# openfheorg/openfhe-boolean-circuit-evaluator

Hardware: AMD Instinct MI355X
Metric: encrypted gate-bootstraps/sec (whole node), AES-128 Bristol ckt STD128 GINX (higher is better)
Workload: dtype u32

## Files before the change

openfhe-boolean-circuit-evaluator_amd/csrc/kernels.hip:

```cpp
#include <hip/hip_runtime.h>

#include <algorithm>
#include <iterator>
#include <utility>

#include "kernels.hpp"

namespace bce {

#include "phase_prof.hpp"
#include "gate_front.hpp"
#include "fused_tail.hpp"
#include "dag_sched.hpp"
#ifdef BCE_PHASE_PROF
__device__ unsigned long long g_phase_prof[BCE_PROF_WAVES * BCE_PROF_SLOTS];
#define BCE_PROF_ARRAY ::bce::g_phase_prof
#endif

__device__ __forceinline__ u32 csub(u32 x, u32 m) { return min(x, x - m); }

__device__ __forceinline__ u32 mul_shoup_lazy(u32 y, uint2 w, u32 Q) {
    u32 qh = __umulhi(w.y, y);
    return w.x * y - qh * Q;
}

__device__ __forceinline__ u64 mad64(u32 a, u32 b, u64 c) {
    u64 r, carry;
    asm("v_mad_u64_u32 %0, %1, %2, %3, %4" : "=v"(r), "=s"(carry) : "v"(a), "v"(b), "v"(c));
    return r;
}
__device__ __forceinline__ u64 mul64(u32 a, u32 b) {
    u64 r, carry;
    asm("v_mad_u64_u32 %0, %1, %2, %3, 0" : "=v"(r), "=s"(carry) : "v"(a), "v"(b));
    return r;
}
__device__ __forceinline__ u32 mul_shoup_lazy3(u32 y, uint2 w, u32 Q) {
    return (u32)mad64(__umulhi(w.y, y), 0u - Q, mul64(y, w.x));
}
__device__ __forceinline__ u64 pair_of(u32 lo) {
    u64 p;
    asm volatile("" : "=v"(p));
    return (p & 0xFFFFFFFF00000000ull) | lo;
}
__device__ __forceinline__ u64 with_lo(u64 pair, u32 lo) { return (pair & 0xFFFFFFFF00000000ull) | lo; }

__device__ __forceinline__ u32 barrett_lazy3(u64 x, u32 Q, u32 shift, u32 mu) {
    return (u32)mad64(__umulhi((u32)(x >> shift), mu), 0u - Q, x);
}

__device__ __forceinline__ u32 barrett_reduce(u64 x, u32 Q, u32 shift, u32 mu) {
    u32 x1 = (u32)(x >> shift);
    u32 qh = __umulhi(x1, mu);
    u32 r = (u32)x - qh * Q;
    r = csub(r, 2 * Q);
    return csub(r, Q);
}

__device__ __forceinline__ u32 barrett_fold(u64 x, u32 c32, u32 Q, u32 shift, u32 mu) {
    return barrett_reduce((u64)(u32)(x >> 32) * c32 + (u32)x, Q, shift, mu);
}


template <int LOGN>
struct Cfg {
    static constexpr int N = 1 << LOGN;
    static constexpr int LE = LOGN - 6;
    static constexpr int E = 1 << LE;
    static constexpr int NP = N + (N >> 6) * 4;
    static constexpr int F2LO = (6 > LE) ? 6 - LE : 0;
    static_assert(LOGN >= 9 && LOGN <= 11, "supported ring sizes: 512, 1024, 2048");
};

template <u32 M>
__device__ __forceinline__ u32 tw_pos(u32 i) {
    if constexpr (M < 64) {
        return M + i;
    } else {
// ... 43 lines not shown
        uint4* p = reinterpret_cast<uint4*>(poly + phys(lane * E));
#pragma unroll
        for (int k = 0; k < E / 4; ++k) p[k] = make_uint4(x[4 * k], x[4 * k + 1], x[4 * k + 2], x[4 * k + 3]);
    } else {
#pragma unroll
        for (int r = 0; r < E; ++r) poly[phys(elem_j<LOGN, LO>(lane, r))] = x[r];
    }
}

template <int LOGN, int LO, int B, bool LAZY>
__device__ __forceinline__ void fwd_stage(u32 (&x)[Cfg<LOGN>::E], u32 lane, const uint2* tw, u32 Q) {
    constexpr int LE = Cfg<LOGN>::LE, E = Cfg<LOGN>::E;
    constexpr int rb = B - LO;
    constexpr u32 m = 1u << (LOGN - 1 - B);
    const u32 hi = (lane >> LO) << (LO + LE - B - 1);
    const u32 Q2 = 2 * Q;
#pragma unroll
    for (int r = 0; r < E; ++r) {
        if (r & (1 << rb)) continue;
        uint2 w = tw[tw_pos<m>(hi | (u32)(r >> (rb + 1)))];
        u32 X = LAZY ? x[r] : csub(x[r], Q2);
        u32 T = mul_shoup_lazy(x[r | (1 << rb)], w, Q);
        x[r] = X + T;
        x[r | (1 << rb)] = X + Q2 - T;
    }
}

template <int LOGN, int LO, int B>
__device__ __forceinline__ void fwd_stage_pair(u64 (&x)[Cfg<LOGN>::E], u32 lane, const uint2* tw, u32 Q) {
    constexpr int LE = Cfg<LOGN>::LE, E = Cfg<LOGN>::E;
    constexpr int rb = B - LO;
    constexpr u32 m = 1u << (LOGN - 1 - B);
    const u32 hi = (lane >> LO) << (LO + LE - B - 1);
    const u32 Q2 = 2 * Q, negQ = 0u - Q;
#pragma unroll
    for (int r = 0; r < E; ++r) {
        if (r & (1 << rb)) continue;
        const uint2 w = tw[tw_pos<m>(hi | (u32)(r >> (rb + 1)))];
        const u32 X = (u32)x[r], Y = (u32)x[r | (1 << rb)];
        const u64 t = mad64(__umulhi(Y, w.y), negQ, mad64(Y, w.x, x[r]));
        x[r | (1 << rb)] = with_lo(x[r | (1 << rb)], (X << 1) + Q2 - (u32)t);
        x[r] = t;
    }
}
template <int LOGN>
__device__ __forceinline__ void fwd_first_stage_pair(const u32 (&x)[Cfg<LOGN>::E], u64 (&xp)[Cfg<LOGN>::E], uint2 w, u32 Q) {
    constexpr int E = Cfg<LOGN>::E, Hh = E / 2;
    const u32 Q2 = 2 * Q, negQ = 0u - Q;
#pragma unroll
    for (int r = 0; r < Hh; ++r) {
        const u32 X = x[r], Y = x[r + Hh];
        const u64 t = mad64(__umulhi(Y, w.y), negQ, mad64(Y, w.x, pair_of(X)));
        xp[r] = t;
        xp[r + Hh] = pair_of((X << 1) + Q2 - (u32)t);
    }
}
template <int LOGN, int LO, int BHI, int BLO>
__device__ __forceinline__ void fwd_stages_pair(u64 (&x)[Cfg<LOGN>::E], u32 lane, const uint2* tw, u32 Q) {
    if constexpr (BHI >= BLO) {
        fwd_stage_pair<LOGN, LO, BHI>(x, lane, tw, Q);
        fwd_stages_pair<LOGN, LO, BHI - 1, BLO>(x, lane, tw, Q);
    }
}
template <int LOGN, int LO>
__device__ __forceinline__ void load_pass_pair(const u32* poly, u32 lane, u64 (&x)[Cfg<LOGN>::E]) {
#pragma unroll
    for (int r = 0; r < Cfg<LOGN>::E; ++r) x[r] = pair_of(poly[phys(elem_j<LOGN, LO>(lane, r))]);
}
__device__ __forceinline__ u32 lm_word(u32 lane, int k) { return (u32)k * 256u + lane * 4u; }
template <int LOGN>
__device__ __forceinline__ void load_lm(const u32* poly, u32 lane, u32 (&x)[Cfg<LOGN>::E]) {
#pragma unroll
    for (int k = 0; k < Cfg<LOGN>::E / 4; ++k) {
        const uint4 v = *reinterpret_cast<const uint4*>(poly + lm_word(lane, k));
        x[4 * k] = v.x; x[4 * k + 1] = v.y; x[4 * k + 2] = v.z; x[4 * k + 3] = v.w;
    }
}
template <int LOGN, int LO>
__device__ __forceinline__ void store_pass_pair(u32* poly, u32 lane, const u64 (&x)[Cfg<LOGN>::E]) {
#pragma unroll
    for (int r = 0; r < Cfg<LOGN>::E; ++r) poly[phys(elem_j<LOGN, LO>(lane, r))] = (u32)x[r];
}

constexpr int GS_CAP = 16;
constexpr int gs_bound(int r, int rb0, int rb) {
    int b = 2;
    for (int s = rb0; s < rb; ++s) {
// ... 98 lines not shown
#pragma unroll
        for (int r = 0; r < C::E; ++r) {
            if constexpr (LAZY) {
                u32 v = x[r] - __umulhi(x[r], mu32) * Q;
                x[r] = csub(csub(v, 2 * Q), Q);
            } else {
                x[r] = csub(csub(x[r], 2 * Q), Q);
            }
        }
    }
    store_pass<LOGN, 0>(poly, lane, x);
    wave_sync();
}

__device__ __forceinline__ void ntt_forward_wave_low8(u32* poly, const uint2* twf, u32 lane, u32 Q) {
    constexpr int LOGN = 10;
    {
        u64 xp[16];
        load_pass_pair<LOGN, 4>(poly, lane, xp);
        fwd_stages_pair<LOGN, 4, 7, 4>(xp, lane, twf, Q);
        store_pass_pair<LOGN, 4>(poly, lane, xp);
    }
    wave_sync();
    u32 x[16];
    u64 xp[16];
    load_pass<LOGN, 0>(poly, lane, x);
    fwd_first_stage_pair<LOGN>(x, xp, twf[tw_pos<64>(lane)], Q);
    fwd_stages_pair<LOGN, 0, 2, 0>(xp, lane, twf, Q);
#pragma unroll
    for (int r = 0; r < 16; ++r) x[r] = (u32)xp[r];
    store_pass<LOGN, 0>(poly, lane, x);
    wave_sync();
}
__device__ __forceinline__ void fwd_bfly_pair(u64& xa, u64& xb, uint2 w, u32 Q) {
    const u32 X = (u32)xa, Y = (u32)xb;
    const u64 t = mad64(__umulhi(Y, w.y), 0u - Q, mad64(Y, w.x, xa));
    xb = with_lo(xb, (X << 1) + 2 * Q - (u32)t);
    xa = t;
}
__device__ __forceinline__ void ntt_forward_half_low8(u32* row, u32 h, const uint2* twf, u32 lane, u32 Q) {
    asm volatile("" : "+v"(lane));
    u64 xp[8];
    {
        const u32 l8 = lane >> 5, j0 = (h << 9) | (l8 << 8) | (lane & 31u);
        u32* const p = row + phys(j0);
#pragma unroll
        for (int r = 0; r < 8; ++r) xp[r] = pair_of(p[(r >> 1) * 68 + (r & 1) * 32]);
        const u32 i7 = (h << 1) | l8;
        const uint2 w7 = twf[tw_pos<4>(i7)];
#pragma unroll
        for (int r = 0; r < 4; ++r) fwd_bfly_pair(xp[r], xp[r + 4], w7, Q);
#pragma unroll
        for (int g = 0; g < 2; ++g) {
            const uint2 w6 = twf[tw_pos<8>((i7 << 1) | g)];
            fwd_bfly_pair(xp[4 * g], xp[4 * g + 2], w6, Q);
            fwd_bfly_pair(xp[4 * g + 1], xp[4 * g + 3], w6, Q);
        }
#pragma unroll
        for (int g = 0; g < 4; ++g) fwd_bfly_pair(xp[2 * g], xp[2 * g + 1], twf[tw_pos<16>((i7 << 2) | g)], Q);
#pragma unroll
        for (int r = 0; r < 8; ++r) p[(r >> 1) * 68 + (r & 1) * 32] = (u32)xp[r];
    }
    wave_sync();
    {
        const u32 lh = lane >> 2, j0 = (h << 9) | (lh << 5) | (lane & 3u);
        u32* const p = row + phys(j0);
#pragma unroll
        for (int r = 0; r < 8; ++r) xp[r] = pair_of(p[4 * r]);
        const u32 i4 = (h << 4) | lh;
        const uint2 w4 = twf[tw_pos<32>(i4)];
#pragma unroll
        for (int r = 0; r < 4; ++r) fwd_bfly_pair(xp[r], xp[r + 4], w4, Q);
#pragma unroll
        for (int g = 0; g < 2; ++g) {
            const uint2 w3 = twf[tw_pos<64>((i4 << 1) | g)];
            fwd_bfly_pair(xp[4 * g], xp[4 * g + 2], w3, Q);
            fwd_bfly_pair(xp[4 * g + 1], xp[4 * g + 3], w3, Q);
        }
#pragma unroll
        for (int g = 0; g < 4; ++g) fwd_bfly_pair(xp[2 * g], xp[2 * g + 1], twf[tw_pos<128>((i4 << 2) | g)], Q);
#pragma unroll
        for (int r = 0; r < 8; ++r) p[4 * r] = (u32)xp[r];
    }
    wave_sync();
    {
        const u32 j0 = (h << 9) | (lane << 3);
        uint4* const p = reinterpret_cast<uint4*>(row + phys(j0));
        const uint4 v0 = p[0], v1 = p[1];
        xp[0] = pair_of(v0.x); xp[1] = pair_of(v0.y); xp[2] = pair_of(v0.z); xp[3] = pair_of(v0.w);
        xp[4] = pair_of(v1.x); xp[5] = pair_of(v1.y); xp[6] = pair_of(v1.z); xp[7] = pair_of(v1.w);
        const u32 i1 = (((h << 6) | lane) << 1);
#pragma unroll
        for (int g = 0; g < 2; ++g) {
            const uint2 w1 = twf[tw_pos<256>(i1 | g)];
            fwd_bfly_pair(xp[4 * g], xp[4 * g + 2], w1, Q);
            fwd_bfly_pair(xp[4 * g + 1], xp[4 * g + 3], w1, Q);
        }
#pragma unroll
        for (int g = 0; g < 4; ++g) fwd_bfly_pair(xp[2 * g], xp[2 * g + 1], twf[tw_pos<512>((i1 << 1) | g)], Q);
        p[0] = make_uint4((u32)xp[0], (u32)xp[1], (u32)xp[2], (u32)xp[3]);
        p[1] = make_uint4((u32)xp[4], (u32)xp[5], (u32)xp[6], (u32)xp[7]);
    }
    wave_sync();
}
__device__ __forceinline__ u64 mad64_su(u32 a, u32 b_uniform, u64 c) {
    u64 r, carry;
    asm("v_mad_u64_u32 %0, %1, %2, %3, %4" : "=v"(r), "=s"(carry) : "v"(a), "s"(b_uniform), "v"(c));
    return r;
}
__device__ __forceinline__ void fwd_bfly_pair_su(u64& xa, u64& xb, uint2 w_uniform, u32 Q) {
    const u32 X = (u32)xa, Y = (u32)xb;
    const u64 t = mad64(__umulhi(Y, w_uniform.y), 0u - Q, mad64_su(Y, w_uniform.x, xa));
    xb = with_lo(xb, (X << 1) + 2 * Q - (u32)t);
    xa = t;
}
template <bool SU>
__device__ __forceinline__ void fwd_pass4_pair(u64 (&x)[4], uint2 wa, uint2 wb0, uint2 wb1, u32 Q) {
    if constexpr (SU) {
        fwd_bfly_pair_su(x[0], x[2], wa, Q); fwd_bfly_pair_su(x[1], x[3], wa, Q);
        fwd_bfly_pair_su(x[0], x[1], wb0, Q); fwd_bfly_pair_su(x[2], x[3], wb1, Q);
    } else {
        fwd_bfly_pair(x[0], x[2], wa, Q); fwd_bfly_pair(x[1], x[3], wa, Q);
        fwd_bfly_pair(x[0], x[1], wb0, Q); fwd_bfly_pair(x[2], x[3], wb1, Q);
    }
}
typedef int v4i __attribute__((ext_vector_type(4)));
__device__ __forceinline__ u32 xb_group(u32 j, u32 g) { return 64u * j + 16u * ((g ^ (0u - (j >> 2))) & 3u); }
template <bool MFMA>
__device__ __forceinline__ void ntt_forward_quarter3(u32* rows, u32 qr, uint2 w7, uint2 w6a, uint2 w6b, const u32* xb,
                                                     const v4i (&A)[4], uint2 w14, const uint2* twf, u32 lane, u32 Q) {
    constexpr int RS = 2 * Cfg<10>::NP;
    u64 xp[3][4];
    auto pass16 = [&](uint2 wa, uint2 wb0, uint2 wb1) {
        const uint4* const p = reinterpret_cast<const uint4*>(rows + 4 * lane);
        uint4 v[3];
#pragma unroll
        for (int k = 0; k < 3; ++k) v[k] = p[k * (RS / 4)];
#pragma unroll
        for (int k = 0; k < 3; ++k) {
            xp[k][0] = ((u64)v[k].y << 32) | v[k].x; xp[k][2] = pair_of(v[k].y);
            xp[k][1] = ((u64)v[k].w << 32) | v[k].z; xp[k][3] = pair_of(v[k].w);
            fwd_pass4_pair<false>(xp[k], wa, wb0, wb1, Q);
        }
    };
    auto store4 = [&](u32 off) {
        u32* const p = rows + off;
#pragma unroll
        for (int k = 0; k < 3; ++k)
#pragma unroll
            for (int r = 0; r < 4; ++r) p[k * RS + 64 * r] = (u32)xp[k][r];
    };
    if constexpr (!MFMA) {
        {
            const u32* const p = rows + lane;
#pragma unroll
            for (int k = 0; k < 3; ++k)
#pragma unroll
                for (int r = 0; r < 4; ++r) xp[k][r] = pair_of(p[k * RS + 68 * r]);
#pragma unroll
            for (int k = 0; k < 3; ++k) fwd_pass4_pair<true>(xp[k], w7, w6a, w6b, Q);
            store4(((lane & 15u) << 2) | ((lane >> 3) & 2u) | (lane >> 5));
        }
        wave_sync();
        {
            const u32 h = lane >> 4;
            const uint2 w5 = twf[tw_pos<16>(4 * qr + h)];
            const uint4 w4 = *reinterpret_cast<const uint4*>(twf + tw_pos<32>(8 * qr + 2 * h));
            pass16(w5, make_uint2(w4.x, w4.y), make_uint2(w4.z, w4.w));
            store4(((lane >> 4) << 4) | ((lane & 3u) << 2) | ((lane >> 1) & 2u) | ((lane >> 3) & 1u));
        }
        wave_sync();
        {
            const u32 h = (((lane >> 2) & 3u) << 2) | (lane >> 4);
            const uint2* const t = twf + tw_pos<64>(16 * qr + h);
            pass16(t[0], t[64], t[128]);
            store4((((lane >> 2) & 3u) << 4) | ((lane >> 4) << 2) | ((lane & 1u) << 1) | ((lane >> 1) & 1u));
        }
    } else {
        {
            const char* const pb = reinterpret_cast<const char*>(xb) + xb_group(lane & 15u, lane >> 4);
            v4i B[3];
#pragma unroll
            for (int k = 0; k < 3; ++k) B[k] = *reinterpret_cast<const v4i*>(pb + 1024 * k);
            const u32 negQ = 0u - Q;
            const v4i c0 = {(int)Q, 0, (int)Q, 0};
#pragma unroll
            for (int i = 0; i < 4; ++i) {
#pragma unroll
                for (int k = 0; k < 3; ++k) {
                    const v4i s = __builtin_amdgcn_mfma_i32_16x16x64_i8(A[i], B[k], c0, 0, 0, 0);
                    const u32 lo = ((u32)s[1] << 7) + (u32)s[0], hi = ((u32)s[3] << 7) + (u32)s[2];
                    xp[k][i] = mad64(__umulhi(hi, w14.y), negQ, mad64_su(hi, w14.x, ((u64)(u32)s[1] << 32) | lo));
                }
            }
            store4(((lane >> 4) << 4) | ((lane & 3u) << 2) | ((lane >> 1) & 2u) | ((lane >> 3) & 1u));
        }
        wave_sync();
        {
            const u32 h = lane >> 2;
            const uint2* const t = twf + tw_pos<64>(16 * qr + h);
            pass16(t[0], t[64], t[128]);
            store4((h << 2) | ((lane & 1u) << 1) | ((lane >> 1) & 1u));
        }
    }
    wave_sync();
    {
        const u32 h = lane & 15u, g = lane >> 4;
        const uint2* const t = twf + 512 + 128 * g + 16 * qr + h;
        pass16(twf[256 + 64 * g + 16 * qr + h], t[0], t[64]);
        uint4* const p = reinterpret_cast<uint4*>(rows + 16 * h + 4 * g + 4 * (h >> 2));
#pragma unroll
        for (int k = 0; k < 3; ++k) p[k * (RS / 4)] = make_uint4((u32)xp[k][0], (u32)xp[k][1], (u32)xp[k][2], (u32)xp[k][3]);
    }
    wave_sync();
}
__device__ __forceinline__ void fwd_bfly(u32& X, u32& Y, uint2 w, u32 Q) {
    const u64 t = mad64(__umulhi(Y, w.y), 0u - Q, mad64(Y, w.x, pair_of(X)));
    Y = (X << 1) + 2 * Q - (u32)t;
    X = (u32)t;
}

template <int LOGN>
__device__ __forceinline__ void ntt_inverse_wave(const u32* src, u32* tmp, const uint2* twi, u32 lane, u32 Q,
                                                 uint2 ninv, uint2 wlast, u32 mu32, u32 (&x)[Cfg<LOGN>::E]) {
    using C = Cfg<LOGN>;
    constexpr int LE = C::LE;
// ... 62 lines not shown

__device__ __forceinline__ u32 redc(u64 x, u32 Q, u32 qn) { return (u32)(mad64((u32)x * qn, Q, x) >> 32); }
template <int LOGN, bool EVENF = false, typename PT>
__device__ __forceinline__ void ginx_mac_tail_redc(const PT& P, __amdgpu_buffer_rsrc_t psi_r2_rsrc, u32 Q, u32 ap, u32 p0,
                                                   const u32* accp, u32* accw, const u64 (&sp)[4], const u64 (&sn)[4],
                                                   u32 (&a)[4]) {
    constexpr u32 N = 1u << LOGN;
    const u32 k0 = __brev(p0) >> (32 - LOGN);
    const u32 ex = ((2 * k0 + 1) * ap) & (2 * N - 1);
    const u32 off = P.r2_off, K = Q + 2 * off, qn = P.qinv_neg;
    u32 mp[4], mn[4];
    const u32 p0r = psi_pow<LOGN>(psi_r2_rsrc, ex, Q), n0r = psi_pow<LOGN>(psi_r2_rsrc, (2 * N - ex) & (2 * N - 1), Q);
    mp[0] = p0r + off;
    mn[0] = n0r + off;
    if constexpr (EVENF) {
        const bool neg = ap & 2u;
        mp[2] = neg ? K - mp[0] : mp[0];
        mn[2] = neg ? K - mn[0] : mn[0];
        mp[1] = mp[0]; mn[1] = mn[0]; mp[3] = mp[2]; mn[3] = mn[2];
    } else {
        const bool odd = ap & 1u;
        const u32 a4 = ap & 3u;
        const uint2 Ia = make_uint2(P.I4[a4], P.I4s[a4]);
        const uint2 Ina = make_uint2(P.I4[(4u - a4) & 3u], P.I4s[(4u - a4) & 3u]);
        mp[2] = csub(mul_shoup_lazy(p0r, Ia, Q), Q) + off;
        mn[2] = csub(mul_shoup_lazy(n0r, Ina, Q), Q) + off;
        mp[1] = odd ? K - mp[0] : mp[0];
        mn[1] = odd ? K - mn[0] : mn[0];
        mp[3] = odd ? K - mp[2] : mp[2];
        mn[3] = odd ? K - mn[2] : mn[2];
    }
    const uint4 a4v = *reinterpret_cast<const uint4*>(accp);
    a[0] = a4v.x; a[1] = a4v.y; a[2] = a4v.z; a[3] = a4v.w;
#pragma unroll
    for (int e = 0; e < 4; ++e) {
        const u32 rp = redc(sp[e], Q, qn), rn = redc(sn[e], Q, qn);
        a[e] = csub(redc(mad64(rn, mn[e], mul64(rp, mp[e])), Q, qn) + a[e], 2 * Q);
    }
    *reinterpret_cast<uint4*>(accw) = make_uint4(a[0], a[1], a[2], a[3]);
}

template <int LOGN, bool LAZY, u32 T, typename PT>
__device__ __forceinline__ void bootstrap_prologue(const PT& P, const bce_gate_desc& g, u32 soff, uint2* twf, u32* acc,
                                                   u32* av, u32 tid, u32 lane, u32 wave) {
    using C = Cfg<LOGN>;
    constexpr int N = C::N, NP = C::NP;
    const u32 Q = P.Q, q = P.q;
    for (u32 i = tid; i < (u32)N; i += T) twf[i] = P.tw_f[i];
    lwe_prepare<T>(P, g, soff, q, av, tid);
    __syncthreads();
    test_polynomial<T, (u32)N>(P, g.op & 0xFFu, q, av[P.n], Q, acc, acc + NP, tid);
    __syncthreads();
    if (wave == 0) ntt_forward_wave<LOGN, LAZY>(acc + NP, twf, lane, Q, P.mu32);
    __syncthreads();
}

template <int LOGN, int DG, bool LAZY, int OCC, bool AP>
__global__ __launch_bounds__(128 * DG, (OCC * 2 * DG + 3) / 4) void k_blind_rotate(
    DevParams P, const bce_gate_desc* __restrict__ descs, u32 n_desc, u32 slot_stride, u32* __restrict__ acc_out) {
    using C = Cfg<LOGN>;
    constexpr int N = C::N, NP = C::NP, E = C::E;
    constexpr u32 R = 2 * DG;
    constexpr u32 T = 64 * R;
    extern __shared__ __align__(16) u32 smem[];
    uint2* twf = reinterpret_cast<uint2*>(smem);
    u32* acc = reinterpret_cast<u32*>(twf + N);
    u32* dct = acc + 2 * NP;
    u32* av = dct + R * NP;

    const u32 tid = threadIdx.x;
    const u32 lane = tid & 63;
// ... 141 lines not shown
                const uint4 d = *reinterpret_cast<const uint4*>(dct + l * NP + pp);
                sn[0] += (u64)d.x * kB[l].x; sn[1] += (u64)d.y * kB[l].y; sn[2] += (u64)d.z * kB[l].z; sn[3] += (u64)d.w * kB[l].w;
            }
#pragma unroll
            for (u32 l = 0; l < H; ++l) {
                const uint4 d = *reinterpret_cast<const uint4*>(dct + (H + l) * NP + pp);
                sn[0] += (u64)d.x * kA[l].x; sn[1] += (u64)d.y * kA[l].y; sn[2] += (u64)d.z * kA[l].z; sn[3] += (u64)d.w * kA[l].w;
            }
            }
            u32 anew[4];
            ginx_mac_tail<LOGN, LAZY>(P, psi_rsrc, Q, ap, Ia, Ina, p0, acc + c * NP + pp, acc + c * NP + pp, sp, sn, anew);
        }
        BCE_PROF_MARK(4);
        __syncthreads();
        BCE_PROF_MARK(5);
    }
    BCE_PROF_FLUSH();

    if (wave < 2) {
        u32 x[E];
        ntt_inverse_wave<LOGN>(acc + wave * NP, dct + wave * NP, twf, lane, Q, ninv, wlast, P.mu32, x);
        u32* out = acc_out + ((size_t)blockIdx.x * 2 + wave) * N;
#pragma unroll
        for (int r = 0; r < E; ++r) out[((u32)r << 6) | lane] = x[r];
    }
}

__device__ __forceinline__ u32 xlay1(u32 p) { return (p & 15u) + 20u * ((p >> 4) & 3u) + 80u * ((p >> 6) & 3u) + 320u * (p >> 8); }
__device__ __forceinline__ u32 xlay2(u32 p) { return (p & 63u) + 80u * ((p >> 6) & 3u) + 320u * (p >> 8); }

__device__ __forceinline__ void inv_pass4(u32 (&x)[4], uint2 fa, uint2 fb, uint2 fc, u32 Q, u32 mu32) {
    const u32 Q2 = 2 * Q;
    const u32 a0 = x[0] + x[1];
    const u32 a1 = mul_shoup_lazy3(x[1] + Q2 - x[0], fa, Q);
    const u32 a2 = x[2] + x[3];
    const u32 a3 = mul_shoup_lazy3(x[3] + Q2 - x[2], fb, Q);
    const u32 b0 = a0 + a2;
    x[2] = mul_shoup_lazy3(a2 + 2 * Q2 - a0, fc, Q);
    const u32 b1 = a1 + a3;
    x[3] = mul_shoup_lazy3(a3 + Q2 - a1, fc, Q);
    x[0] = b0 - __umulhi(b0, mu32) * Q;
    x[1] = csub(b1, Q2);
}
__device__ __forceinline__ void inv_pass4_last(u32 (&x)[4], uint2 fa, uint2 fb, uint2 ninv, uint2 wlast, u32 Q) {
    const u32 Q2 = 2 * Q;
    const u32 a0 = x[0] + x[1];
    const u32 a1 = mul_shoup_lazy3(x[1] + Q2 - x[0], fa, Q);
    const u32 a2 = x[2] + x[3];
    const u32 a3 = mul_shoup_lazy3(x[3] + Q2 - x[2], fb, Q);
    x[0] = csub(mul_shoup_lazy3(a0 + a2, ninv, Q), Q);
    x[2] = csub(mul_shoup_lazy3(a0 + 2 * Q2 - a2, wlast, Q), Q);
    x[1] = csub(mul_shoup_lazy3(a1 + a3, ninv, Q), Q);
    x[3] = csub(mul_shoup_lazy3(a1 + Q2 - a3, wlast, Q), Q);
}

template <bool REGTW>
struct SplitInv {
    u32 a0, x0, l1, s1, l2, s2, l3, s3, t;
    uint2 fa[REGTW ? 5 : 1], fb[REGTW ? 5 : 1], fc[REGTW ? 4 : 1];
    u32 ia[REGTW ? 1 : 4], ic[REGTW ? 1 : 4];
};
template <bool REGTW>
__device__ __forceinline__ void split_inv_setup(SplitInv<REGTW>& S, const uint2* twf, u32 t) {
    S.t = t;
    S.a0 = phys(4 * t);
    const u32 wb = 48u * (t >> 6);
    S.x0 = S.a0 + wb;
    const u32 pb1 = ((t >> 2) << 4) | (t & 3u), pb2 = ((t >> 4) << 6) | (t & 15u), pb3 = ((t >> 6) << 8) | (t & 63u);
    S.l1 = phys(pb1) + wb; S.s1 = xlay1(pb1);
    S.l2 = xlay1(pb2); S.s2 = xlay2(pb2);
    S.l3 = xlay2(pb3); S.s3 = 320u * (t >> 6) + (t & 63u);
    const u32 u0 = t, u1 = t >> 2, u2 = t >> 4, u3 = t >> 6;
    if constexpr (REGTW) {
        S.fa[0] = twf[tw_pos<512>(511 - 2 * u0)]; S.fb[0] = twf[tw_pos<512>(510 - 2 * u0)]; S.fc[0] = twf[tw_pos<256>(255 - u0)];
        S.fa[1] = twf[tw_pos<128>(127 - 2 * u1)]; S.fb[1] = twf[tw_pos<128>(126 - 2 * u1)]; S.fc[1] = twf[tw_pos<64>(63 - u1)];
        S.fa[2] = twf[tw_pos<32>(31 - 2 * u2)];   S.fb[2] = twf[tw_pos<32>(30 - 2 * u2)];   S.fc[2] = twf[tw_pos<16>(15 - u2)];
        S.fa[3] = twf[tw_pos<8>(7 - 2 * u3)];     S.fb[3] = twf[tw_pos<8>(6 - 2 * u3)];     S.fc[3] = twf[tw_pos<4>(3 - u3)];
        S.fa[4] = twf[tw_pos<2>(1)];              S.fb[4] = twf[tw_pos<2>(0)];
    } else {
        S.ia[0] = tw_pos<512>(511 - 2 * u0); S.ic[0] = tw_pos<256>(255 - u0);
        S.ia[1] = tw_pos<128>(127 - 2 * u1); S.ic[1] = tw_pos<64>(63 - u1);
        S.ia[2] = tw_pos<32>(31 - 2 * u2);   S.ic[2] = tw_pos<16>(15 - u2);
        S.ia[3] = tw_pos<8>(7 - 2 * u3);     S.ic[3] = tw_pos<4>(3 - u3);
    }
}
template <bool REGTW, int K>
// ... 130 lines not shown
    const u32 psel0 = 0x0c0c0400u, psel1 = 0x05040100u;
    const u32 mc = tid / (N / 4), mp0 = (tid % (N / 4)) * 4, mpp = phys(mp0);
    const u32 dig0 = phys(S.t);
    const uint2 w9 = twf[1], w8a = twf[2], w8b = twf[3];
    uint2 q7 = make_uint2(0, 0), q6a = q7, q6b = q7;
    if constexpr (QUNITS && !MFMA) {
        const uint2 a = twf[tw_pos<4>(wave & 3u)], b = twf[tw_pos<8>(2 * (wave & 3u))], d = twf[tw_pos<8>(2 * (wave & 3u) + 1)];
        q7 = make_uint2(__builtin_amdgcn_readfirstlane(a.x), __builtin_amdgcn_readfirstlane(a.y));
        q6a = make_uint2(__builtin_amdgcn_readfirstlane(b.x), __builtin_amdgcn_readfirstlane(b.y));
        q6b = make_uint2(__builtin_amdgcn_readfirstlane(d.x), __builtin_amdgcn_readfirstlane(d.y));
    }
    {
        const uint4 v = *reinterpret_cast<const uint4*>(accc + S.a0);
        u32 a[4] = {v.x, v.y, v.z, v.w};
        split_pass0(S, twf, a, xa, Q, P.mu32);
    }

    BCE_PROF_INIT();
    const u32 nsteps = AP ? n * P.dR : n;
    u32 cb = 0;
    if constexpr (WPS >= 4) __builtin_amdgcn_s_setprio(2);
    for (u32 step = 0; step < nsteps; ++step) {
        u32 ap = 0, rowb;
        if constexpr (!AP) {
            ap = ginx_exponent(P, q, av[step]);
            if (ap == 0) continue;
            rowb = step * (2 * rgsw * 4);
        } else {
            const u32 i = step / P.dR, kd = step - i * P.dR;
            const u32 a0 = ap_digit(P, q, av[i], kd);
            if (a0 == 0) continue;
            rowb = (((i * P.baseR + a0) * P.dR + kd) * rgsw) * 4u;
        }
        uint4 kA[R], kB[R];
        v4i mA[4];
        auto request_rows = [&](auto kc) {
            constexpr u32 k = decltype(kc)::value - 1, G = PR / 4;
            BCE_PROF_MARK(8 + k);
#pragma unroll
            for (u32 l = k * G; l < (k + 1) * G; ++l) {
                kA[l] = bsk_row(rsrc, tid * 16u, rowb + l * (2 * N * 4));
                if constexpr (!AP) kB[l] = bsk_row(rsrc, tid * 16u, rowb + (rgsw + l * 2 * N) * 4);
            }
            if constexpr (MFMA && k == 3) {
#pragma unroll
                for (u32 v = 0; v < 4; ++v) mA[v] = __builtin_bit_cast(v4i, bsk_row(mrsrc, lane * 16u, ((wave & 3u) * 4u + v) * 1024u));
            }
        };
        {
            u32 x[4], u[4];
            split_inverse_rest(S, twf, xa, xb, Q, P.mu32, ninv, wlast, x, request_rows);
#pragma unroll
            for (int r = 0; r < 4; ++r) u[r] = x[r] + ((x[r] < Qh) ? off : offm);
            if constexpr (MFMA) {
#pragma unroll
                for (int r = 0; r < 4; ++r) u[r] ^= off;
            }
#pragma unroll
            for (u32 l = FOLD ? 1 : 0; l < (u32)DG; ++l) {
                if constexpr (MFMA) {
                    const u32 e01 = __builtin_amdgcn_perm((u32)__builtin_amdgcn_sbfe((int)u[1], l * gb, gb), (u32)__builtin_amdgcn_sbfe((int)u[0], l * gb, gb), psel0);
                    const u32 e23 = __builtin_amdgcn_perm((u32)__builtin_amdgcn_sbfe((int)u[3], l * gb, gb), (u32)__builtin_amdgcn_sbfe((int)u[2], l * gb, gb), psel0);
                    const u32 d = __builtin_amdgcn_perm(e23, e01, psel1);
                    const u32 G = S.t >> 4;
                    xbm[(3 * c + l - 1) * 256 + (xb_group(S.t & 15u, G >> 2) >> 2) + (G & 3u)] = d;
                    continue;
                }
                u32 v[4];
#pragma unroll
                for (int r = 0; r < 4; ++r) v[r] = __builtin_amdgcn_ubfe(u[r], l * gb, gb) + bias;
                fwd_bfly(v[0], v[2], w9, Q);
                fwd_bfly(v[1], v[3], w9, Q);
                fwd_bfly(v[0], v[1], w8a, Q);
                fwd_bfly(v[2], v[3], w8b, Q);
#pragma unroll
                for (int r = 0; r < 4; ++r) dct[(2 * l + c) * NP + dig0 + 272 * r] = v[r];
            }
        }
        BCE_PROF_MARK(0);
        block_sync_lds();
        BCE_PROF_MARK(1);
        if constexpr (WPS >= 4) { if (FOLD && wave >= 4) __builtin_amdgcn_s_setprio(1); else __builtin_amdgcn_s_setprio(0); }
#ifndef BCE_SKIP_FWD
        if constexpr (QUNITS) {
            ntt_forward_quarter3<MFMA>(dct + (2 + c) * NP + 272u * (wave & 3u), wave & 3u, q7, q6a, q6b, xbm + 3 * c * 256, mA,
                                       make_uint2(P.w14, P.w14s), twf, lane, Q);
        } else if constexpr (FOLD) {
            if (wave < 4) ntt_forward_wave_low8(dct + (2 + wave) * NP, twf, lane, Q);
            else ntt_forward_half_low8(dct + (6 + ((wave - 4) >> 1)) * NP, (wave - 4) & 1u, twf, lane, Q);
        } else {
            ntt_forward_wave_low8(dct + wave * NP, twf, lane, Q);
        }
#endif
        if constexpr (WPS >= 4) __builtin_amdgcn_s_setprio(2);
        BCE_PROF_MARK(2);
        if constexpr (PR < R) {
#pragma unroll
            for (u32 l = PR; l < R; ++l) kA[l] = bsk_row(rsrc, tid * 16u, rowb + l * (2 * N * 4));
#pragma unroll
            for (u32 l = PR; l < R; ++l) if constexpr (!AP) kB[l] = bsk_row(rsrc, tid * 16u, rowb + (rgsw + l * 2 * N) * 4);
        }
        block_sync_lds();
        BCE_PROF_MARK(3);
        {
            u64 sp[4] = {0, 0, 0, 0}, sn[4] = {0, 0, 0, 0};
#pragma unroll
            for (u32 l = 0; l < R; ++l) {
#ifdef BCE_SKIP_MAC
                const uint4 d = make_uint4(l + tid, l, tid, 1u);
#else
                const uint4 d = *reinterpret_cast<const uint4*>((FOLD && l < 2 ? acc + cb : dct) + l * NP + mpp);
#endif
                sp[0] += (u64)d.x * kA[l].x; sp[1] += (u64)d.y * kA[l].y; sp[2] += (u64)d.z * kA[l].z; sp[3] += (u64)d.w * kA[l].w;
                if constexpr (!AP) {
                    sn[0] += (u64)d.x * kB[l].x; sn[1] += (u64)d.y * kB[l].y; sn[2] += (u64)d.z * kB[l].z; sn[3] += (u64)d.w * kB[l].w;
                }
            }
            u32 anew[4];
            const u32* const accr = acc + cb + mc * NP + mpp;
            u32* const accw = acc + (FOLD ? 2 * NP - cb : 0) + mc * NP + mpp;
            if constexpr (AP) {
#pragma unroll
                for (int e = 0; e < 4; ++e) anew[e] = barrett_fold(sp[e], P.c32, Q, P.red_shift, P.red_mu);
                *reinterpret_cast<uint4*>(accw) = make_uint4(anew[0], anew[1], anew[2], anew[3]);
            } else {
                ginx_mac_tail_redc<LOGN, V::EVENF>(P, psi_rsrc, Q, ap, mp0, accr, accw, sp, sn, anew);
            }
            if constexpr (FOLD) cb = 2 * NP - cb;
            split_pass0(S, twf, anew, xa, Q, P.mu32);
        }
        BCE_PROF_MARK(4);
        wave_sync();
        BCE_PROF_MARK(5);
    }
    BCE_PROF_FLUSH();
    {
        u32 x[4];
        split_inverse_rest(S, twf, xa, xb, Q, P.mu32, ninv, wlast, x, [](auto) {});
        if (acc_out) {
            u32* out = acc_out + ((size_t)boot * 2 + c) * N + S.t;
#pragma unroll
            for (int r = 0; r < 4; ++r) out[256 * r] = x[r];
        }
        if constexpr (FUSE) {
#pragma unroll
            for (int r = 0; r < 4; ++r) acc[c * N + S.t + 256 * r] = x[r];
        }
    }
    if constexpr (FUSE) {
        if constexpr (WPS >= 4) __builtin_amdgcn_s_setprio(0);
        __syncthreads();
        fused_tail_outputs<T, PERSIST>(P, g, soff, acc, dct, reinterpret_cast<u64*>(dct + ((N * P.dKS + 3) & ~3u)), boot, dbg_lweN, dbg_ks);
    }
}

template <class V>
__global__ __launch_bounds__(V::T, V::WPS) void k_blind_rotate_lat(DevParams P, const bce_gate_desc* __restrict__ descs, u32 n_desc,
                                                                   u32 slot_stride, u32* __restrict__ acc_out,
                                                                   u32* __restrict__ dbg_lweN, u32* __restrict__ dbg_ks) {
    extern __shared__ __align__(16) u32 smem[];
    lat_bootstrap<V, false>(P, descs[blockIdx.x % n_desc], (blockIdx.x / n_desc) * slot_stride, blockIdx.x, smem, acc_out, dbg_lweN, dbg_ks);
}
// ... 487 lines not shown
```

Before: 193,600.

## Batch NTT butterflies into grouped multiplies for instruction-level parallelism

Replaces the inline-asm v_mad_u64_u32 helpers with plain 64-bit C multiplies, wrapped in an empty asm barrier so the 64-bit pair stays in vector registers. Forward butterflies, inverse passes and the MAC tail reduction are regrouped so that 4 or 6 independent mulhi/mad chains are issued together instead of one dependent chain at a time. The modulus is pinned to a scalar register, and a scheduling barrier is added inside the MAC loop. The aim is to hide multiply latency and let the compiler use the carry-free mad form, at the cost of higher register pressure and a possible loss of occupancy.

```diff
diff --git a/openfhe-boolean-circuit-evaluator_amd/csrc/kernels.hip b/openfhe-boolean-circuit-evaluator_amd/csrc/kernels.hip
--- a/openfhe-boolean-circuit-evaluator_amd/csrc/kernels.hip
+++ b/openfhe-boolean-circuit-evaluator_amd/csrc/kernels.hip
@@ -24,16 +24,16 @@
     return w.x * y - qh * Q;
 }
 
-__device__ __forceinline__ u64 mad64(u32 a, u32 b, u64 c) {
-    u64 r, carry;
-    asm("v_mad_u64_u32 %0, %1, %2, %3, %4" : "=v"(r), "=s"(carry) : "v"(a), "v"(b), "v"(c));
+__device__ __forceinline__ u64 keep_pair(u64 r) {
+    asm volatile("" :: "v"(r));
     return r;
 }
-__device__ __forceinline__ u64 mul64(u32 a, u32 b) {
-    u64 r, carry;
-    asm("v_mad_u64_u32 %0, %1, %2, %3, 0" : "=v"(r), "=s"(carry) : "v"(a), "v"(b));
-    return r;
-}
+__device__ __forceinline__ u64 mad64(u32 a, u32 b, u64 c) { return keep_pair((u64)a * b + c); }
+__device__ __forceinline__ u32 block_local(u32 s) {
+    asm volatile("" : "+s"(s));
+    return s;
+}
+__device__ __forceinline__ u64 mul64(u32 a, u32 b) { return (u64)a * b; }
 __device__ __forceinline__ u32 mul_shoup_lazy3(u32 y, uint2 w, u32 Q) {
     return (u32)mad64(__umulhi(w.y, y), 0u - Q, mul64(y, w.x));
 }
@@ -43,6 +43,35 @@
     return (p & 0xFFFFFFFF00000000ull) | lo;
 }
 __device__ __forceinline__ u64 with_lo(u64 pair, u32 lo) { return (pair & 0xFFFFFFFF00000000ull) | lo; }
+
+template <int K>
+__device__ __forceinline__ void mul_shoup_lazy3_group(const u32 (&y)[K], const uint2 (&w)[K], u32 Q, u32 (&r)[K]) {
+    u32 qh[K];
+    u64 t[K];
+#pragma unroll
+    for (int k = 0; k < K; ++k) qh[k] = __umulhi(w[k].y, y[k]);
+#pragma unroll
+    for (int k = 0; k < K; ++k) t[k] = mul64(y[k], w[k].x);
+#pragma unroll
+    for (int k = 0; k < K; ++k) r[k] = (u32)mad64(qh[k], 0u - Q, t[k]);
+}
+template <int K>
+__device__ __forceinline__ void fwd_bfly_group(u64* x, const int (&ia)[K], const int (&ib)[K], const uint2 (&w)[K], u32 Q) {
+    u32 qh[K];
+    u64 t[K];
+#pragma unroll
+    for (int k = 0; k < K; ++k) qh[k] = __umulhi((u32)x[ib[k]], w[k].y);
+#pragma unroll
+    for (int k = 0; k < K; ++k) t[k] = mad64((u32)x[ib[k]], w[k].x, x[ia[k]]);
+#pragma unroll
+    for (int k = 0; k < K; ++k) t[k] = mad64(qh[k], 0u - Q, t[k]);
+#pragma unroll
+    for (int k = 0; k < K; ++k) {
+        const u32 X = (u32)x[ia[k]];
+        x[ib[k]] = with_lo(x[ib[k]], (X << 1) + 2 * Q - (u32)t[k]);
+        x[ia[k]] = t[k];
+    }
+}
 
 __device__ __forceinline__ u32 barrett_lazy3(u64 x, u32 Q, u32 shift, u32 mu) {
     return (u32)mad64(__umulhi((u32)(x >> shift), mu), 0u - Q, x);
@@ -152,27 +181,42 @@
     constexpr int rb = B - LO;
     constexpr u32 m = 1u << (LOGN - 1 - B);
     const u32 hi = (lane >> LO) << (LO + LE - B - 1);
-    const u32 Q2 = 2 * Q, negQ = 0u - Q;
-#pragma unroll
-    for (int r = 0; r < E; ++r) {
-        if (r & (1 << rb)) continue;
-        const uint2 w = tw[tw_pos<m>(hi | (u32)(r >> (rb + 1)))];
-        const u32 X = (u32)x[r], Y = (u32)x[r | (1 << rb)];
-        const u64 t = mad64(__umulhi(Y, w.y), negQ, mad64(Y, w.x, x[r]));
-        x[r | (1 << rb)] = with_lo(x[r | (1 << rb)], (X << 1) + Q2 - (u32)t);
-        x[r] = t;
+    constexpr int G = E / 2 < 4 ? E / 2 : 4;
+#pragma unroll
+    for (int g = 0; g < E / 2; g += G) {
+        int ia[G], ib[G];
+        uint2 w[G];
+#pragma unroll
+        for (int k = 0; k < G; ++k) {
+            const int b = g + k;
+            const int r = ((b >> rb) << (rb + 1)) | (b & ((1 << rb) - 1));
+            ia[k] = r;
+            ib[k] = r | (1 << rb);
+            w[k] = tw[tw_pos<m>(hi | (u32)(r >> (rb + 1)))];
+        }
+        fwd_bfly_group<G>(x, ia, ib, w, Q);
     }
 }
 template <int LOGN>
 __device__ __forceinline__ void fwd_first_stage_pair(const u32 (&x)[Cfg<LOGN>::E], u64 (&xp)[Cfg<LOGN>::E], uint2 w, u32 Q) {
     constexpr int E = Cfg<LOGN>::E, Hh = E / 2;
     const u32 Q2 = 2 * Q, negQ = 0u - Q;
-#pragma unroll
-    for (int r = 0; r < Hh; ++r) {
-        const u32 X = x[r], Y = x[r + Hh];
-        const u64 t = mad64(__umulhi(Y, w.y), negQ, mad64(Y, w.x, pair_of(X)));
-        xp[r] = t;
-        xp[r + Hh] = pair_of((X << 1) + Q2 - (u32)t);
+    constexpr int G = Hh < 4 ? Hh : 4;
+#pragma unroll
+    for (int g = 0; g < Hh; g += G) {
+        u32 qh[G];
+        u64 t[G];
+#pragma unroll
+        for (int k = 0; k < G; ++k) qh[k] = __umulhi(x[g + k + Hh], w.y);
+#pragma unroll
+        for (int k = 0; k < G; ++k) t[k] = mad64(x[g + k + Hh], w.x, pair_of(x[g + k]));
+#pragma unroll
+        for (int k = 0; k < G; ++k) t[k] = mad64(qh[k], negQ, t[k]);
+#pragma unroll
+        for (int k = 0; k < G; ++k) {
+            xp[g + k] = t[k];
+            xp[g + k + Hh] = pair_of((x[g + k] << 1) + Q2 - (u32)t[k]);
+        }
     }
 }
 template <int LOGN, int LO, int BHI, int BLO>
@@ -337,12 +381,6 @@
     store_pass<LOGN, 0>(poly, lane, x);
     wave_sync();
 }
-__device__ __forceinline__ void fwd_bfly_pair(u64& xa, u64& xb, uint2 w, u32 Q) {
-    const u32 X = (u32)xa, Y = (u32)xb;
-    const u64 t = mad64(__umulhi(Y, w.y), 0u - Q, mad64(Y, w.x, xa));
-    xb = with_lo(xb, (X << 1) + 2 * Q - (u32)t);
-    xa = t;
-}
 __device__ __forceinline__ void ntt_forward_half_low8(u32* row, u32 h, const uint2* twf, u32 lane, u32 Q) {
     asm volatile("" : "+v"(lane));
     u64 xp[8];
@@ -353,16 +391,13 @@
         for (int r = 0; r < 8; ++r) xp[r] = pair_of(p[(r >> 1) * 68 + (r & 1) * 32]);
         const u32 i7 = (h << 1) | l8;
         const uint2 w7 = twf[tw_pos<4>(i7)];
-#pragma unroll
-        for (int r = 0; r < 4; ++r) fwd_bfly_pair(xp[r], xp[r + 4], w7, Q);
-#pragma unroll
-        for (int g = 0; g < 2; ++g) {
-            const uint2 w6 = twf[tw_pos<8>((i7 << 1) | g)];
-            fwd_bfly_pair(xp[4 * g], xp[4 * g + 2], w6, Q);
-            fwd_bfly_pair(xp[4 * g + 1], xp[4 * g + 3], w6, Q);
-        }
-#pragma unroll
-        for (int g = 0; g < 4; ++g) fwd_bfly_pair(xp[2 * g], xp[2 * g + 1], twf[tw_pos<16>((i7 << 2) | g)], Q);
+        fwd_bfly_group<4>(xp, {0, 1, 2, 3}, {4, 5, 6, 7}, {w7, w7, w7, w7}, Q);
+        {
+            const uint2 w6a = twf[tw_pos<8>(i7 << 1)], w6b = twf[tw_pos<8>((i7 << 1) | 1)];
+            fwd_bfly_group<4>(xp, {0, 1, 4, 5}, {2, 3, 6, 7}, {w6a, w6a, w6b, w6b}, Q);
+        }
+        fwd_bfly_group<4>(xp, {0, 2, 4, 6}, {1, 3, 5, 7}, {twf[tw_pos<16>(i7 << 2)], twf[tw_pos<16>((i7 << 2) | 1)],
+                                                           twf[tw_pos<16>((i7 << 2) | 2)], twf[tw_pos<16>((i7 << 2) | 3)]}, Q);
 #pragma unroll
         for (int r = 0; r < 8; ++r) p[(r >> 1) * 68 + (r & 1) * 32] = (u32)xp[r];
     }
@@ -374,16 +409,13 @@
         for (int r = 0; r < 8; ++r) xp[r] = pair_of(p[4 * r]);
         const u32 i4 = (h << 4) | lh;
         const uint2 w4 = twf[tw_pos<32>(i4)];
-#pragma unroll
-        for (int r = 0; r < 4; ++r) fwd_bfly_pair(xp[r], xp[r + 4], w4, Q);
-#pragma unroll
-        for (int g = 0; g < 2; ++g) {
-            const uint2 w3 = twf[tw_pos<64>((i4 << 1) | g)];
-            fwd_bfly_pair(xp[4 * g], xp[4 * g + 2], w3, Q);
-            fwd_bfly_pair(xp[4 * g + 1], xp[4 * g + 3], w3, Q);
-        }
-#pragma unroll
-        for (int g = 0; g < 4; ++g) fwd_bfly_pair(xp[2 * g], xp[2 * g + 1], twf[tw_pos<128>((i4 << 2) | g)], Q);
+        fwd_bfly_group<4>(xp, {0, 1, 2, 3}, {4, 5, 6, 7}, {w4, w4, w4, w4}, Q);
+        {
+            const uint2 w3a = twf[tw_pos<64>(i4 << 1)], w3b = twf[tw_pos<64>((i4 << 1) | 1)];
+            fwd_bfly_group<4>(xp, {0, 1, 4, 5}, {2, 3, 6, 7}, {w3a, w3a, w3b, w3b}, Q);
+        }
+        fwd_bfly_group<4>(xp, {0, 2, 4, 6}, {1, 3, 5, 7}, {twf[tw_pos<128>(i4 << 2)], twf[tw_pos<128>((i4 << 2) | 1)],
+                                                           twf[tw_pos<128>((i4 << 2) | 2)], twf[tw_pos<128>((i4 << 2) | 3)]}, Q);
 #pragma unroll
         for (int r = 0; r < 8; ++r) p[4 * r] = (u32)xp[r];
     }
@@ -395,39 +427,21 @@
         xp[0] = pair_of(v0.x); xp[1] = pair_of(v0.y); xp[2] = pair_of(v0.z); xp[3] = pair_of(v0.w);
         xp[4] = pair_of(v1.x); xp[5] = pair_of(v1.y); xp[6] = pair_of(v1.z); xp[7] = pair_of(v1.w);
         const u32 i1 = (((h << 6) | lane) << 1);
-#pragma unroll
-        for (int g = 0; g < 2; ++g) {
-            const uint2 w1 = twf[tw_pos<256>(i1 | g)];
-            fwd_bfly_pair(xp[4 * g], xp[4 * g + 2], w1, Q);
-            fwd_bfly_pair(xp[4 * g + 1], xp[4 * g + 3], w1, Q);
-        }
-#pragma unroll
-        for (int g = 0; g < 4; ++g) fwd_bfly_pair(xp[2 * g], xp[2 * g + 1], twf[tw_pos<512>((i1 << 1) | g)], Q);
+        {
+            const uint2 w1a = twf[tw_pos<256>(i1)], w1b = twf[tw_pos<256>(i1 | 1)];
+            fwd_bfly_group<4>(xp, {0, 1, 4, 5}, {2, 3, 6, 7}, {w1a, w1a, w1b, w1b}, Q);
+        }
+        fwd_bfly_group<4>(xp, {0, 2, 4, 6}, {1, 3, 5, 7}, {twf[tw_pos<512>(i1 << 1)], twf[tw_pos<512>((i1 << 1) | 1)],
+                                                           twf[tw_pos<512>((i1 << 1) | 2)], twf[tw_pos<512>((i1 << 1) | 3)]}, Q);
         p[0] = make_uint4((u32)xp[0], (u32)xp[1], (u32)xp[2], (u32)xp[3]);
         p[1] = make_uint4((u32)xp[4], (u32)xp[5], (u32)xp[6], (u32)xp[7]);
     }
     wave_sync();
 }
-__device__ __forceinline__ u64 mad64_su(u32 a, u32 b_uniform, u64 c) {
-    u64 r, carry;
-    asm("v_mad_u64_u32 %0, %1, %2, %3, %4" : "=v"(r), "=s"(carry) : "v"(a), "s"(b_uniform), "v"(c));
-    return r;
-}
-__device__ __forceinline__ void fwd_bfly_pair_su(u64& xa, u64& xb, uint2 w_uniform, u32 Q) {
-    const u32 X = (u32)xa, Y = (u32)xb;
-    const u64 t = mad64(__umulhi(Y, w_uniform.y), 0u - Q, mad64_su(Y, w_uniform.x, xa));
-    xb = with_lo(xb, (X << 1) + 2 * Q - (u32)t);
-    xa = t;
-}
-template <bool SU>
-__device__ __forceinline__ void fwd_pass4_pair(u64 (&x)[4], uint2 wa, uint2 wb0, uint2 wb1, u32 Q) {
-    if constexpr (SU) {
-        fwd_bfly_pair_su(x[0], x[2], wa, Q); fwd_bfly_pair_su(x[1], x[3], wa, Q);
-        fwd_bfly_pair_su(x[0], x[1], wb0, Q); fwd_bfly_pair_su(x[2], x[3], wb1, Q);
-    } else {
-        fwd_bfly_pair(x[0], x[2], wa, Q); fwd_bfly_pair(x[1], x[3], wa, Q);
-        fwd_bfly_pair(x[0], x[1], wb0, Q); fwd_bfly_pair(x[2], x[3], wb1, Q);
-    }
+__device__ __forceinline__ void fwd_pass4_pair3(u64 (&x)[3][4], uint2 wa, uint2 wb0, uint2 wb1, u32 Q) {
+    u64* const f = &x[0][0];
+    fwd_bfly_group<6>(f, {0, 1, 4, 5, 8, 9}, {2, 3, 6, 7, 10, 11}, {wa, wa, wa, wa, wa, wa}, Q);
+    fwd_bfly_group<6>(f, {0, 2, 4, 6, 8, 10}, {1, 3, 5, 7, 9, 11}, {wb0, wb1, wb0, wb1, wb0, wb1}, Q);
 }
 typedef int v4i __attribute__((ext_vector_type(4)));
 __device__ __forceinline__ u32 xb_group(u32 j, u32 g) { return 64u * j + 16u * ((g ^ (0u - (j >> 2))) & 3u); }
@@ -445,8 +459,8 @@
         for (int k = 0; k < 3; ++k) {
             xp[k][0] = ((u64)v[k].y << 32) | v[k].x; xp[k][2] = pair_of(v[k].y);
             xp[k][1] = ((u64)v[k].w << 32) | v[k].z; xp[k][3] = pair_of(v[k].w);
-            fwd_pass4_pair<false>(xp[k], wa, wb0, wb1, Q);
-        }
+        }
+        fwd_pass4_pair3(xp, wa, wb0, wb1, Q);
     };
     auto store4 = [&](u32 off) {
         u32* const p = rows + off;
@@ -462,8 +476,7 @@
             for (int k = 0; k < 3; ++k)
 #pragma unroll
                 for (int r = 0; r < 4; ++r) xp[k][r] = pair_of(p[k * RS + 68 * r]);
-#pragma unroll
-            for (int k = 0; k < 3; ++k) fwd_pass4_pair<true>(xp[k], w7, w6a, w6b, Q);
+            fwd_pass4_pair3(xp, w7, w6a, w6b, Q);
             store4(((lane & 15u) << 2) | ((lane >> 3) & 2u) | (lane >> 5));
         }
         wave_sync();
@@ -491,12 +504,21 @@
             const v4i c0 = {(int)Q, 0, (int)Q, 0};
 #pragma unroll
             for (int i = 0; i < 4; ++i) {
+                v4i s[3];
+                u32 hi[3], qh[3];
+                u64 t[3];
+#pragma unroll
+                for (int k = 0; k < 3; ++k) s[k] = __builtin_amdgcn_mfma_i32_16x16x64_i8(A[i], B[k], c0, 0, 0, 0);
 #pragma unroll
                 for (int k = 0; k < 3; ++k) {
-                    const v4i s = __builtin_amdgcn_mfma_i32_16x16x64_i8(A[i], B[k], c0, 0, 0, 0);
-                    const u32 lo = ((u32)s[1] << 7) + (u32)s[0], hi = ((u32)s[3] << 7) + (u32)s[2];
-                    xp[k][i] = mad64(__umulhi(hi, w14.y), negQ, mad64_su(hi, w14.x, ((u64)(u32)s[1] << 32) | lo));
+                    t[k] = ((u64)(u32)s[k][1] << 32) | (((u32)s[k][1] << 7) + (u32)s[k][0]);
+                    hi[k] = ((u32)s[k][3] << 7) + (u32)s[k][2];
+                    qh[k] = __umulhi(hi[k], w14.y);
                 }
+#pragma unroll
+                for (int k = 0; k < 3; ++k) t[k] = mad64(hi[k], w14.x, t[k]);
+#pragma unroll
+                for (int k = 0; k < 3; ++k) xp[k][i] = mad64(qh[k], negQ, t[k]);
             }
             store4(((lane >> 4) << 4) | ((lane & 3u) << 2) | ((lane >> 1) & 2u) | ((lane >> 3) & 1u));
         }
@@ -625,11 +647,16 @@
     }
     const uint4 a4v = *reinterpret_cast<const uint4*>(accp);
     a[0] = a4v.x; a[1] = a4v.y; a[2] = a4v.z; a[3] = a4v.w;
-#pragma unroll
-    for (int e = 0; e < 4; ++e) {
-        const u32 rp = redc(sp[e], Q, qn), rn = redc(sn[e], Q, qn);
-        a[e] = csub(redc(mad64(rn, mn[e], mul64(rp, mp[e])), Q, qn) + a[e], 2 * Q);
-    }
+    u32 rp[4], rn[4];
+    u64 t[4];
+#pragma unroll
+    for (int e = 0; e < 4; ++e) rp[e] = redc(sp[e], Q, qn);
+#pragma unroll
+    for (int e = 0; e < 4; ++e) rn[e] = redc(sn[e], Q, qn);
+#pragma unroll
+    for (int e = 0; e < 4; ++e) t[e] = mad64(rn[e], mn[e], mul64(rp[e], mp[e]));
+#pragma unroll
+    for (int e = 0; e < 4; ++e) a[e] = csub(redc(t[e], Q, qn) + a[e], 2 * Q);
     *reinterpret_cast<uint4*>(accw) = make_uint4(a[0], a[1], a[2], a[3]);
 }
 
@@ -837,26 +864,26 @@
 __device__ __forceinline__ void inv_pass4(u32 (&x)[4], uint2 fa, uint2 fb, uint2 fc, u32 Q, u32 mu32) {
     const u32 Q2 = 2 * Q;
     const u32 a0 = x[0] + x[1];
-    const u32 a1 = mul_shoup_lazy3(x[1] + Q2 - x[0], fa, Q);
     const u32 a2 = x[2] + x[3];
-    const u32 a3 = mul_shoup_lazy3(x[3] + Q2 - x[2], fb, Q);
+    u32 a[2], b[2];
+    mul_shoup_lazy3_group<2>({x[1] + Q2 - x[0], x[3] + Q2 - x[2]}, {fa, fb}, Q, a);
     const u32 b0 = a0 + a2;
-    x[2] = mul_shoup_lazy3(a2 + 2 * Q2 - a0, fc, Q);
-    const u32 b1 = a1 + a3;
-    x[3] = mul_shoup_lazy3(a3 + Q2 - a1, fc, Q);
+    const u32 b1 = a[0] + a[1];
+    mul_shoup_lazy3_group<2>({a2 + 2 * Q2 - a0, a[1] + Q2 - a[0]}, {fc, fc}, Q, b);
+    x[2] = b[0];
+    x[3] = b[1];
     x[0] = b0 - __umulhi(b0, mu32) * Q;
     x[1] = csub(b1, Q2);
 }
 __device__ __forceinline__ void inv_pass4_last(u32 (&x)[4], uint2 fa, uint2 fb, uint2 ninv, uint2 wlast, u32 Q) {
     const u32 Q2 = 2 * Q;
     const u32 a0 = x[0] + x[1];
-    const u32 a1 = mul_shoup_lazy3(x[1] + Q2 - x[0], fa, Q);
     const u32 a2 = x[2] + x[3];
-    const u32 a3 = mul_shoup_lazy3(x[3] + Q2 - x[2], fb, Q);
-    x[0] = csub(mul_shoup_lazy3(a0 + a2, ninv, Q), Q);
-    x[2] = csub(mul_shoup_lazy3(a0 + 2 * Q2 - a2, wlast, Q), Q);
-    x[1] = csub(mul_shoup_lazy3(a1 + a3, ninv, Q), Q);
-    x[3] = csub(mul_shoup_lazy3(a1 + Q2 - a3, wlast, Q), Q);
+    u32 a[2], r[4];
+    mul_shoup_lazy3_group<2>({x[1] + Q2 - x[0], x[3] + Q2 - x[2]}, {fa, fb}, Q, a);
+    mul_shoup_lazy3_group<4>({a0 + a2, a[0] + a[1], a0 + 2 * Q2 - a2, a[0] + Q2 - a[1]}, {ninv, ninv, wlast, wlast}, Q, r);
+#pragma unroll
+    for (int k = 0; k < 4; ++k) x[k] = csub(r[k], Q);
 }
 
 template <bool REGTW>
@@ -1053,6 +1080,7 @@
             if (a0 == 0) continue;
             rowb = (((i * P.baseR + a0) * P.dR + kd) * rgsw) * 4u;
         }
+        const u32 Qs = block_local(Q);
         uint4 kA[R], kB[R];
         v4i mA[4];
         auto request_rows = [&](auto kc) {
@@ -1070,7 +1098,7 @@
         };
         {
             u32 x[4], u[4];
-            split_inverse_rest(S, twf, xa, xb, Q, P.mu32, ninv, wlast, x, request_rows);
+            split_inverse_rest(S, twf, xa, xb, Qs, P.mu32, ninv, wlast, x, request_rows);
 #pragma unroll
             for (int r = 0; r < 4; ++r) u[r] = x[r] + ((x[r] < Qh) ? off : offm);
             if constexpr (MFMA) {
@@ -1090,10 +1118,10 @@
                 u32 v[4];
 #pragma unroll
                 for (int r = 0; r < 4; ++r) v[r] = __builtin_amdgcn_ubfe(u[r], l * gb, gb) + bias;
-                fwd_bfly(v[0], v[2], w9, Q);
-                fwd_bfly(v[1], v[3], w9, Q);
-                fwd_bfly(v[0], v[1], w8a, Q);
-                fwd_bfly(v[2], v[3], w8b, Q);
+                fwd_bfly(v[0], v[2], w9, Qs);
+                fwd_bfly(v[1], v[3], w9, Qs);
+                fwd_bfly(v[0], v[1], w8a, Qs);
+                fwd_bfly(v[2], v[3], w8b, Qs);
 #pragma unroll
                 for (int r = 0; r < 4; ++r) dct[(2 * l + c) * NP + dig0 + 272 * r] = v[r];
             }
@@ -1105,12 +1133,12 @@
 #ifndef BCE_SKIP_FWD
         if constexpr (QUNITS) {
             ntt_forward_quarter3<MFMA>(dct + (2 + c) * NP + 272u * (wave & 3u), wave & 3u, q7, q6a, q6b, xbm + 3 * c * 256, mA,
-                                       make_uint2(P.w14, P.w14s), twf, lane, Q);
+                                       make_uint2(P.w14, P.w14s), twf, lane, Qs);
         } else if constexpr (FOLD) {
-            if (wave < 4) ntt_forward_wave_low8(dct + (2 + wave) * NP, twf, lane, Q);
-            else ntt_forward_half_low8(dct + (6 + ((wave - 4) >> 1)) * NP, (wave - 4) & 1u, twf, lane, Q);
+            if (wave < 4) ntt_forward_wave_low8(dct + (2 + wave) * NP, twf, lane, Qs);
+            else ntt_forward_half_low8(dct + (6 + ((wave - 4) >> 1)) * NP, (wave - 4) & 1u, twf, lane, Qs);
         } else {
-            ntt_forward_wave_low8(dct + wave * NP, twf, lane, Q);
+            ntt_forward_wave_low8(dct + wave * NP, twf, lane, Qs);
         }
 #endif
         if constexpr (WPS >= 4) __builtin_amdgcn_s_setprio(2);
@@ -1136,19 +1164,20 @@
                 if constexpr (!AP) {
                     sn[0] += (u64)d.x * kB[l].x; sn[1] += (u64)d.y * kB[l].y; sn[2] += (u64)d.z * kB[l].z; sn[3] += (u64)d.w * kB[l].w;
                 }
+                if (l == 1) __builtin_amdgcn_sched_barrier(0);
             }
             u32 anew[4];
             const u32* const accr = acc + cb + mc * NP + mpp;
             u32* const accw = acc + (FOLD ? 2 * NP - cb : 0) + mc * NP + mpp;
             if constexpr (AP) {
 #pragma unroll
-                for (int e = 0; e < 4; ++e) anew[e] = barrett_fold(sp[e], P.c32, Q, P.red_shift, P.red_mu);
+                for (int e = 0; e < 4; ++e) anew[e] = barrett_fold(sp[e], P.c32, Qs, P.red_shift, P.red_mu);
                 *reinterpret_cast<uint4*>(accw) = make_uint4(anew[0], anew[1], anew[2], anew[3]);
             } else {
-                ginx_mac_tail_redc<LOGN, V::EVENF>(P, psi_rsrc, Q, ap, mp0, accr, accw, sp, sn, anew);
+                ginx_mac_tail_redc<LOGN, V::EVENF>(P, psi_rsrc, Qs, ap, mp0, accr, accw, sp, sn, anew);
             }
             if constexpr (FOLD) cb = 2 * NP - cb;
-            split_pass0(S, twf, anew, xa, Q, P.mu32);
+            split_pass0(S, twf, anew, xa, Qs, P.mu32);
         }
         BCE_PROF_MARK(4);
         wave_sync();
```

Result: slower. 183,800 (-5.0%).
